# jfjell/Octree-Raymarcher

Measured on AMD Instinct MI355X. Metric: Mrays/s (primary+shadow) at 1920x1080, depth-12 SVO, higher is better.
Workload: dtype f32; 1 GPU; c3_1080p_depth12_4x1x4_shadow; depth_per_chunk=12, chunksize=128, nodes=99473656, bricks=34206642, hbm_pool_bytes=11087035656, kernel=auto, launches_in_flight=2, frames_per_launch=16, frames_in_flight=32, gather=False, partition=single, ranks_seen=1, launcher=single process

## Files before the change

### octree-raymarcher_amd/csrc/kernel_stack.hip.h

```cpp
#pragma once
#include "march.hip.h"
#include "step_asm.hip.h"

namespace svo {

constexpr int CW_ESCAPE_PENDING = (int)0x80000000;
enum : int { M_DONE = 0, M_WORLD = 1, M_HIT = 2, M_TREE = 3, M_TWIG = 4 };

constexpr int VOTE_WORLD = 8;
constexpr int VOTE_HIT = 16;
constexpr int VOTE_BUSY = 24;
constexpr int CREEP_SERIOUS = 6;
constexpr int CREEP_LANES = 8;
#define SVO_LIKELY(x) __builtin_expect(!!(x), 1)
#define SVO_UNLIKELY(x) __builtin_expect(!!(x), 0)
constexpr int STEP_EXTRA = 4;
constexpr int STEP_LANES = 8;
constexpr int DRAIN_STEPS = 8;
#ifndef SVO_SURE_MISS_WHEN
#define SVO_SURE_MISS_WHEN __builtin_amdgcn_readfirstlane(more ? 0 : 1)
#endif

__device__ __forceinline__ float recip_pow2(float x) { return __uint_as_float(0x7F000000u - __float_as_uint(x)); }

__device__ __forceinline__ int chunk_index_pow2(const TraceArgs &A, V3 p)
{
    float qx = p.x * A.inv_chunksize, qy = p.y * A.inv_chunksize, qz = p.z * A.inv_chunksize;
    if (qx < 0.0f) qx -= 1.0f;
    if (qy < 0.0f) qy -= 1.0f;
    if (qz < 0.0f) qz -= 1.0f;
    const int ix = (int)qx, iy = (int)qy, iz = (int)qz;
    const int rx = ix - A.ccm[0], ry = iy - A.ccm[1], rz = iz - A.ccm[2];
    int mx = A.cbase[0] + rx, my = A.cbase[1] + ry, mz = A.cbase[2] + rz;
    mx -= (mx >= A.dimw) ? A.dimw : 0; mx += (mx < 0) ? A.dimw : 0;
    my -= (my >= A.dimh) ? A.dimh : 0; my += (my < 0) ? A.dimh : 0;
    mz -= (mz >= A.dimd) ? A.dimd : 0; mz += (mz < 0) ? A.dimd : 0;
    return my * A.dimw * A.dimd + mz * A.dimw + mx;
}

__device__ __forceinline__ V3 cube_normal_pow2(V3 s, V3 lo, float size, float eps)
{
    const V3 hi = lo + size;
    const V3 c = (lo + hi) * 0.5f;
    const V3 p = s - c;
    const float d = fabsf(lo.x - hi.x) * 0.5f;
    const float invd = recip_pow2(d);
    const float b = 1.0f + eps;
    const float ix = (float)(int)((p.x * invd) * b), iy = (float)(int)((p.y * invd) * b), iz = (float)(int)((p.z * invd) * b);
    const float dot = ix * ix + iy * iy + iz * iz;
    float inv;
    if (dot == 1.0f) inv = 1.0f;
    else if (dot == 2.0f) inv = __uint_as_float(0x3F3504F3u);
    else if (dot == 3.0f) inv = __uint_as_float(0x3F13CD3Au);
    else inv = 1.0f / sqrtf(dot);
    return mk(ix * inv, iy * inv, iz * inv);
}

__device__ __forceinline__ uint32_t child_slot(int ux, int uy, int uz, int sh)
{
    const uint32_t bx = __builtin_amdgcn_ubfe((uint32_t)ux, (uint32_t)sh, 1u);
    const uint32_t by = __builtin_amdgcn_ubfe((uint32_t)uy, (uint32_t)sh, 1u);
    const uint32_t bz = __builtin_amdgcn_ubfe((uint32_t)uz, (uint32_t)sh, 1u);
    return ((bz << 1) + by) * 2u + bx;
}
__device__ __forceinline__ uint32_t ld_node(const uint32_t *pool, uint32_t boff)
{
    return *reinterpret_cast<const uint32_t *>(reinterpret_cast<const char *>(pool) + (size_t)boff);
}
constexpr uint32_t WIDE_PAYLOAD = (1u << 25) - 1u;
__device__ __forceinline__ uint32_t wide_slot(int ux, int uy, int uz, int sh)
{
    const uint32_t bx = __builtin_amdgcn_ubfe((uint32_t)ux, (uint32_t)sh, 2u);
    const uint32_t by = __builtin_amdgcn_ubfe((uint32_t)uy, (uint32_t)sh, 2u);
    const uint32_t bz = __builtin_amdgcn_ubfe((uint32_t)uz, (uint32_t)sh, 2u);
    return (bz << 4) | (by << 2) | bx;
}
__device__ __forceinline__ bool is_branch(uint32_t word) { return (int32_t)word < (int32_t)0xC0000000; }

__device__ __forceinline__ TraceArgs args_reloaded()
{
    auto p = __builtin_amdgcn_kernarg_segment_ptr();
    asm volatile("" : "+s"(p));
    TraceArgs T;
    __builtin_memcpy(&T, p, sizeof T);
    return T;
}
__device__ __forceinline__ FrameCam camera_reloaded(int f)
{
    auto p = __builtin_amdgcn_kernarg_segment_ptr();
    asm volatile("" : "+s"(p));
    FrameCam c;
    __builtin_memcpy(&c, (decltype(p))((const char __attribute__((address_space(4))) *)p + __builtin_offsetof(TraceArgs, cams) + (size_t)f * sizeof(FrameCam)), sizeof c);
    return c;
}

__device__ __noinline__ float brick_layer_first_touch(int k, V3 a, V3 b, V3 g, V3 bmin, float r, unsigned long long mask)
{
    const float ak = k == 0 ? a.x : k == 1 ? a.y : a.z, bk = k == 0 ? b.x : k == 1 ? b.y : b.z, mk_ = k == 0 ? bmin.x : k == 1 ? bmin.y : bmin.z;
    const float au = k == 0 ? a.y : k == 1 ? a.z : a.x, av = k == 0 ? a.z : k == 1 ? a.x : a.y;
    const float gu = k == 0 ? g.y : k == 1 ? g.z : g.x, gv = k == 0 ? g.z : k == 1 ? g.x : g.y;
    const float mu = k == 0 ? bmin.y : k == 1 ? bmin.z : bmin.x, mv = k == 0 ? bmin.z : k == 1 ? bmin.x : bmin.y;
    const int su = k == 0 ? 4 : k == 1 ? 16 : 1, sv = k == 0 ? 16 : k == 1 ? 1 : 4;
    const float delta = r * 0.0625f;
    bool ok = (ak == mk_) & (bk < 0.0f);
    ok &= (mu >= 4.0f * r) & (mv >= 4.0f * r) & (delta >= (fabsf(mu) + fabsf(mv) + 8.0f * r) * 0x1p-21f);
    ok = ok && fabsf(gu) < 1.0e30f && fabsf(gv) < 1.0e30f;
    if (!ok) return -1.0f;
    const float u0 = au - mu, v0 = av - mv;
    float first = __uint_as_float(0x7F800000u);
    bool clean = true;
    for (int cv = 0; cv < 4; ++cv) {
        const float va = ((float)cv * r - delta - v0) * gv, vb = ((float)(cv + 1) * r + delta - v0) * gv;
        const float v_in = fminf(va, vb), v_out = fmaxf(va, vb);
        for (int cu = 0; cu < 4; ++cu) {
            const bool occupied = (mask >> (cu * su + cv * sv)) & 1ull;
            const float ua = ((float)cu * r - delta - u0) * gu, ub = ((float)(cu + 1) * r + delta - u0) * gu;
            const float s_in = fmaxf(fmaxf(fminf(ua, ub), v_in), 0.0f), s_out = fminf(fmaxf(ua, ub), v_out);
            clean &= (s_in == s_in) & (s_out == s_out);
            first = (occupied & (s_in <= s_out)) ? fminf(first, s_in) : first;
        }
    }
    return clean ? first * (1.0f - 0x1p-18f) : -1.0f;
}

__device__ __forceinline__ void note_tile_cost(int outk, uint32_t steps)
{
    const TraceArgs T = args_reloaded();
    if (!T.tile_cost) return;
    const int k = outk & 0x7FFFFFFF;
    int tile, frame = 0;
    if (T.from_camera) {
        const int per = T.w * T.h;
        frame = k / per;
        const int r = k - frame * per;
        const int ly = r / T.w, lx = r - ly * T.w;
        tile = (ly / TILE_H) * T.tiles_per_row + lx / TILE_W;
    } else tile = k >> 6;
    atomicMax(&T.tile_cost[((size_t)frame * (size_t)T.ntiles + (size_t)tile) * 2 + (outk < 0 ? 1 : 0)], steps);
}

template <bool GLSL>
__device__ __forceinline__ bool past_far_end(int mode, float t, float tt_saved, float tw, float eps, float far)
{
    const float tt = mode == M_TWIG ? tt_saved : t;
    return (mode == M_TREE || mode == M_TWIG) && tw + (GLSL ? tt : tt - eps) >= far;
}

template <int MAXLV, int REFILL, int WAVES_PER_SIMD, bool BIG, bool GLSL, bool SEG = false>
__global__ __launch_bounds__(64, WAVES_PER_SIMD) void k_trace_stack(TraceArgs A)
{
    __shared__ uint32_t stk[MAXLV / 2 + 1][64];
    __shared__ float tile_ray[SEG ? 12 : 11][64];
    constexpr int CHUNK_TAB = (BIG && MAXLV <= 10) ? 128 : 64;
    __shared__ uint32_t chunk_tab[6][CHUNK_TAB];
    stk[0][threadIdx.x] = 0u;
    const int lane = threadIdx.x;
    const bool want_cost = A.tile_cost != nullptr;
    const int n_chunks = A.dimw * A.dimh * A.dimd;
    const bool chunks_in_lds = n_chunks <= CHUNK_TAB;
    if (chunks_in_lds)
        for (int i = lane; i < n_chunks; i += 64) {
            const DevWide ch = A.wchunks[i];
            chunk_tab[0][i] = __float_as_uint(ch.bmin[0]); chunk_tab[1][i] = __float_as_uint(ch.bmin[1]); chunk_tab[2][i] = __float_as_uint(ch.bmin[2]);
            chunk_tab[3][i] = ch.levels; chunk_tab[4][i] = ch.wide_off; chunk_tab[5][i] = (uint32_t)ch.twig_off;
        }
    __syncthreads();
#ifdef SVO_STACK_TIMING
    const unsigned long long t_begin = __builtin_amdgcn_s_memrealtime();
    unsigned n_iters = 0, n_tree_lanes = 0, n_twig_lanes = 0, n_world_lanes = 0;
    unsigned n_world_runs = 0, n_hit_runs = 0, n_refill = 0, n_tilegen = 0, n_fix = 0;
    unsigned n_lane_twig = 0;
    unsigned n_lane_busy = 0;
    unsigned n_creep_runs = 0, n_creep_rounds = 0, n_dbg = 0;
    unsigned n_wsteps = 0, n_lsteps = 0, n_hit_wait = 0, n_dead_wait = 0, n_wsteps_b = 0, n_lsteps_b = 0, n_world_wait = 0, n_twig_b = 0;
#endif
    [[maybe_unused]] StepStats step_stats;

    const V3 wlo = ld3(A.worldmin), whi = ld3(A.worldmax);
    const V3 sdir = ld3(A.sdir);
    const V3 sg = recip(sdir);
    const float eps = A.eps;
    const bool eps_pow2 = (__float_as_uint(eps) & 0x807FFFFFu) == 0u && __float_as_uint(eps) >= 0x00800000u && __float_as_uint(eps) < 0x7F800000u;
    const float csize = A.chunksize;

    const int tr_cols = A.tiles_per_row;
    const int tr_rows = A.ntiles / (tr_cols > 0 ? tr_cols : 1);
    const bool by_cols = tr_cols >= TILE_REGIONS;
    const int reg_q = (by_cols ? tr_cols : tr_rows) / TILE_REGIONS, reg_rem = (by_cols ? tr_cols : tr_rows) % TILE_REGIONS;
    int region = (int)(__builtin_amdgcn_s_getreg(20 | (0 << 6) | (3 << 11)) & (TILE_REGIONS - 1));
    int regions_left = TILE_REGIONS;
    int tile_first = 0;
    int tile_next = 64;
    bool more = true;
    unsigned rays_marched = 0;

    int mode = M_DONE;
    int outk = 0;
    V3 alpha = mk(0, 0, 0), beta = mk(0, 0, 1), g = mk(0, 0, 0);
    float tw = 0.0f;
    [[maybe_unused]] float far = __uint_as_float(0x7F800000u);
    int cw = 0;
    uint32_t guard = 0;
    V3 O = mk(0, 0, 0), Blo = mk(0, 0, 0);
    float res = 1.0f, t = 0.0f;
    int cnt = 0;
    float tt_saved = 0.0f, t_miss = 0.0f;
    int it_saved = 0;
    V3 clo = mk(0, 0, 0);
    WideRef<BIG> wide_b = 0;
    auto ld_wide = [&](uint32_t e) -> uint32_t {
        if constexpr (BIG) return *reinterpret_cast<const uint32_t *>((size_t)wide_b + ((size_t)e << 2));
        else return ld_node(A.wide, wide_b + (e << 2));
    };
    uint32_t twig_off = 0;
    int levels = 0, ci = -1;
    int pux = 0, puy = 0, puz = 0, valid = 0, plev = 0;
    unsigned long long bmask = 0;
#ifndef SVO_CXX_STEP
    float bsize = 0.0f, res_tree = 1.0f;
    int nw_chunk = 1;
    const uint32_t lds_lane = (uint32_t)(size_t)(__attribute__((address_space(3))) uint32_t *)&stk[0][lane];
    StepUniform SU;
    SU.csize = csize; SU.eps = eps; SU.eps2 = 2.0f * eps; SU.cap_twig = A.cap_twig; SU.wide = A.wide; SU.mask = A.mask; SU.descend_shift = MAXLV <= 10 ? DESCEND_SHIFT_SHALLOW : DESCEND_SHIFT_DEEP;
#endif
    int creepn = 0;
    for (;;) {
        unsigned long long dead = __ballot(mode == M_DONE);
        while (more && __popcll(dead) >= REFILL) {
            if (tile_next >= 64) {
                int t32 = -1, tcol = 0, trow = 0, tframe = 0;
                const uint32_t *order = args_reloaded().tile_order;
                if (order) {
                    regions_left = 0;
                    unsigned long long tix = 0;
                    if (lane == 0) tix = atomicAdd(&A.work[WORK_CURSOR0], 1ull);
                    int t = __builtin_amdgcn_readfirstlane((int)tix);
                    if (t < A.ntiles * A.nframes) {
                        tframe = t / A.ntiles; t -= tframe * A.ntiles;
                        t32 = (int)order[t];
                        if ((uint32_t)t32 >= (uint32_t)A.ntiles) { t32 = 0; tframe = -1; }
                        trow = t32 / tr_cols; tcol = t32 - trow * tr_cols;
                    }
                }
                while (regions_left > 0) {
                    const int span = reg_q + (region < reg_rem ? 1 : 0);
                    const int first = region * reg_q + (region < reg_rem ? region : reg_rem);
                    const int count = span * (by_cols ? tr_rows : tr_cols);
                    unsigned long long tix = 0;
                    if (lane == 0) tix = atomicAdd(&A.work[WORK_CURSOR0 + region], 1ull);
                    int t = __builtin_amdgcn_readfirstlane((int)tix);
                    if (t < count * A.nframes) {
                        if (A.nframes > 1) { tframe = t / count; t -= tframe * count; }
                        if (by_cols) { trow = t / span; tcol = first + (t - trow * span); }
                        else { trow = first + t / tr_cols; tcol = t % tr_cols; }
                        t32 = trow * tr_cols + tcol;
                        break;
                    }
                    region = (region + 1) & (TILE_REGIONS - 1);
                    --regions_left;
                }
                if (t32 < 0) { more = false; break; }
                tile_first = t32 * 64;
                tile_next = 0;
#ifdef SVO_STACK_TIMING
                ++n_tilegen;
#endif
                {
                    const TraceArgs T = args_reloaded();
                    const int id = tile_first + lane;
                    bool ok;
                    int k = -1;
                    V3 o = mk(0, 0, 0), d = mk(0, 0, 1);
                    if (T.from_camera) {
                        const int lx = tcol * TILE_W + (lane & (TILE_W - 1));
                        const int ly = trow * TILE_H + lane / TILE_W;
                        ok = (lx < T.w) & (ly < T.h) & (tframe >= 0);
                        k = (tframe * T.h + ly) * T.w + lx;
                        int px = 0, py = 0;
                        if (ok) local_to_pixel(T, lx, ly, px, py);
                        if (ok && (py >= T.imgh || px >= T.imgw)) { store_miss(A.out, k, 0); ok = false; }
                        if (ok) camera_ray(camera_reloaded(tframe), T.imgw, T.imgh, px, py, o, d);
                    } else {
                        ok = id < T.n && tframe >= 0;
                        k = id;
                        if (ok) { o = ld3(T.origins + 3 * (long long)id); d = ld3(T.dirs + 3 * (long long)id); }
                        if constexpr (SEG) tile_ray[11][lane] = ok ? T.tmax[id] : 0.0f;
                    }
                    const V3 gg = recip(d);
                    float t0 = 0.0f;
                    if (ok) {
                        bool hit = true;
                        if (!inside(o, wlo, whi)) t0 = (GLSL ? enter_glsl(o, gg, wlo, whi, hit) : enter(o, d, wlo, whi, hit)) + eps;
                        rays_marched++;
                        if (!hit) { store_miss(A.out, k, 0); ok = false; }
                    }
                    tile_ray[0][lane] = o.x; tile_ray[1][lane] = o.y; tile_ray[2][lane] = o.z;
                    tile_ray[3][lane] = d.x; tile_ray[4][lane] = d.y; tile_ray[5][lane] = d.z;
                    tile_ray[6][lane] = gg.x; tile_ray[7][lane] = gg.y; tile_ray[8][lane] = gg.z;
                    tile_ray[9][lane] = t0;
                    tile_ray[10][lane] = __int_as_float(ok ? k : -1);
                    __syncthreads();
                }
            }
#ifdef SVO_STACK_TIMING
            ++n_refill;
#endif
            const int rank = (int)__builtin_amdgcn_mbcnt_hi((unsigned)(dead >> 32), __builtin_amdgcn_mbcnt_lo((unsigned)dead, 0u));
            const int avail = 64 - tile_next;
            if (mode == M_DONE && rank < avail) {
                const int slot = tile_next + rank;
                const int k = __float_as_int(tile_ray[10][slot]);
                if (k >= 0) {
                    outk = k;
                    alpha = mk(tile_ray[0][slot], tile_ray[1][slot], tile_ray[2][slot]);
                    beta = mk(tile_ray[3][slot], tile_ray[4][slot], tile_ray[5][slot]);
                    g = mk(tile_ray[6][slot], tile_ray[7][slot], tile_ray[8][slot]);
                    tw = tile_ray[9][slot];
                    if constexpr (SEG) far = tile_ray[11][slot];
                    cw = 0; guard = 0; creepn = 0;
                    mode = M_WORLD;
                }
            }
            const int ndead = __popcll(dead);
            tile_next += (ndead < avail) ? ndead : avail;
            __syncthreads();
            dead = __ballot(mode == M_DONE);
        }
        if (dead == ~0ull) break;
#ifdef SVO_STACK_TIMING
        ++n_iters;
        n_tree_lanes += __popcll(__ballot(mode == M_TREE)); n_twig_lanes += __popcll(__ballot(mode == M_TWIG));
        n_world_lanes += __popcll(__ballot(mode == M_WORLD));
#endif

        const int n_busy = __popcll(__ballot(mode == M_TREE || mode == M_TWIG));
        const int n_world = __popcll(__ballot(mode == M_WORLD));
        const int n_hit = __popcll(__ballot(mode == M_HIT));
        const bool run_world = n_world > 0 && (n_world >= VOTE_WORLD || n_busy < VOTE_BUSY ||
                                               __ballot(mode == M_WORLD && creepn <= -CREEP_SERIOUS) != 0ull);
        const bool run_hit = n_hit > 0 && (n_hit >= VOTE_HIT || n_busy < VOTE_BUSY);

        if (SVO_UNLIKELY(mode != M_DONE && mode != M_HIT && ++guard > STEP_GUARD)) {
            if (outk < 0) store_flags(A.out, outk & 0x7FFFFFFF, SVO_HIT_FLAG | SVO_SHADOW_TRACED | SVO_ERR_FLAG | (A.normal_mode == SVO_NORMAL_FACE ? (uint32_t)SVO_FACE_NORMAL : 0u));
            else store_miss(A.out, outk, SVO_ERR_FLAG);
            mode = M_DONE;
        }

#ifdef SVO_STACK_TIMING
        n_world_runs += run_world; n_hit_runs += run_hit;
#endif
        if (run_world && mode == M_WORLD) {
            if (cw < 0) {
                cw &= ~CW_ESCAPE_PENDING;
                if constexpr (GLSL) tw += guarded(escape(O, g, clo, clo + csize), eps) + eps;
                else tw += escape(O, g, clo, clo + csize) + eps;
            }
            bool miss = cw >= A.cap_chunk;
            if constexpr (SEG) miss |= (GLSL ? tw : tw - eps) >= far;
            if (!miss) {
                cw++;
                const V3 p = alpha + beta * tw;
                miss = !inside(p, wlo, whi);
                if (!miss) {
                    const int ci_new = chunk_index_pow2(A, p);
                    if (ci_new != ci) { valid = 0; pux = 0; puy = 0; puz = 0; }
                    ci = ci_new;
                    uint32_t ch_levels, ch_wide, ch_twig;
                    if (chunks_in_lds) {
                        clo = mk(__uint_as_float(chunk_tab[0][ci]), __uint_as_float(chunk_tab[1][ci]), __uint_as_float(chunk_tab[2][ci]));
                        ch_levels = chunk_tab[3][ci]; ch_wide = chunk_tab[4][ci]; ch_twig = chunk_tab[5][ci];
                    } else {
                        const DevWide ch = A.wchunks[ci];
                        clo = ld3(ch.bmin);
                        ch_levels = ch.levels; ch_wide = ch.wide_off; ch_twig = (uint32_t)ch.twig_off;
                    }
                    bool contained = inside(p, clo, clo + csize);
                    if (GLSL && !contained) tw += guarded(escape(p, g, clo, clo + csize), eps) + eps;
                    else miss = !contained;
                    if (contained) {
                        if constexpr (BIG) wide_b = (unsigned long long)(size_t)A.wide + ((unsigned long long)ch_wide << 8);
                        else wide_b = ch_wide << 8;
                        twig_off = ch_twig;
                        levels = (int)ch_levels;
                        O = p; t = 0.0f; cnt = A.cap_tree;
                        Blo = clo;
                        res = csize * __uint_as_float((uint32_t)(127 - levels) << 23);
#ifndef SVO_CXX_STEP
                        bsize = csize; res_tree = res; nw_chunk = levels ? (levels + 1) >> 1 : 1;
#endif
                        mode = M_TREE;
                    }
                }
            }
            if (miss) {
                if (outk >= 0) store_miss(A.out, outk, 0);
                if (want_cost) note_tile_cost(outk, guard);
                mode = M_DONE;
            }
        }

        int pass = 0;
        const int fixed_steps = (n_busy >= STEP_LANES && __ballot(creepn > 0 || creepn <= -4 * CREEP_SERIOUS) == 0ull) ? STEP_EXTRA : 0;
        for (;;) {
#ifdef SVO_STACK_TIMING
        n_lane_twig += mode == M_TWIG ? (pass == 0 ? 1u + (unsigned)fixed_steps : (unsigned)DRAIN_STEPS) : 0u;
        n_lane_busy += (mode == M_TREE || mode == M_TWIG) ? (pass == 0 ? 1u + (unsigned)fixed_steps : (unsigned)DRAIN_STEPS) : 0u;
        { const int nm = __popcll(__ballot(mode == M_TREE || mode == M_TWIG)); n_wsteps += nm > 0; n_lsteps += nm; if (more) { n_wsteps_b += nm > 0; n_lsteps_b += nm; n_hit_wait += __popcll(__ballot(mode == M_HIT)); n_dead_wait += __popcll(__ballot(mode == M_DONE)); n_world_wait += __popcll(__ballot(mode == M_WORLD)); n_twig_b += __popcll(__ballot(mode == M_TWIG)); } }
#endif
#ifndef SVO_CXX_STEP
        const int nsteps = pass == 0 ? 1 + fixed_steps : DRAIN_STEPS;
        const int sure_miss = SVO_SURE_MISS_WHEN;
        march_steps_asm<BIG, GLSL>(mode, O, Blo, bsize, res, t, cnt, tt_saved, t_miss, it_saved, tw, cw, pux, puy, puz, valid, plev, bmask, creepn,
                                   beta, g, clo, alpha, levels, nw_chunk, res_tree, wide_b, twig_off, lds_lane, SU, nsteps | (sure_miss << 16), step_stats);
        pass += nsteps - 1;
#else
        if (mode == M_TREE || mode == M_TWIG) {
            enum : int { S_LEAVE = 0, S_ADVANCE = 1, S_ENTER = 2, S_HIT_LEAF = 3, S_HIT_CELL = 4, S_BAD = 5 };
            const bool twig = mode == M_TWIG;
            const float Bsize = twig ? res * 4.0f : csize, inv_res = recip_pow2(res);
            const int crept = creepn < 0 ? -creepn : creepn;
            creepn = -crept;
            bool leave = cnt <= 0;
            cnt -= 1;
            const V3 p = O + beta * t;
            leave |= !inside(p, Blo, Blo + Bsize);
            const float fx = (p.x - Blo.x) * inv_res, fy = (p.y - Blo.y) * inv_res, fz = (p.z - Blo.z) * inv_res;
            int ux = (int)fx, uy = (int)fy, uz = (int)fz;
#ifdef SVO_STACK_TIMING
            n_fix += __ballot(!twig && ((fx == (float)ux) | (fy == (float)uy) | (fz == (float)uz))) != 0;
#endif
            if (SVO_UNLIKELY(!twig && ((fx == (float)ux) | (fy == (float)uy) | (fz == (float)uz)))) {
                const int nmax = (1 << levels) - 1;
                ux = ux > nmax ? nmax : ux; uy = uy > nmax ? nmax : uy; uz = uz > nmax ? nmax : uz;
                ux -= (Blo.x + (float)ux * res > p.x) ? 1 : 0;
                uy -= (Blo.y + (float)uy * res > p.y) ? 1 : 0;
                uz -= (Blo.z + (float)uz * res > p.z) ? 1 : 0;
            }
            if (twig) leave |= (ux > 3) | (uy > 3) | (uz > 3);

            int what = S_LEAVE;
            int low = 0;
            uint32_t payload = 0;
            if (SVO_LIKELY(!leave)) {
                if (!twig) {
                    const uint32_t diff = (uint32_t)((ux ^ pux) | (uy ^ puy) | (uz ^ puz));
                    const int nw = levels ? (levels + 1) >> 1 : 1;
                    const int hb = 32 - __clz((int)(diff | 1u));
                    const int keep = nw - ((hb + 1) >> 1);
                    int k;
                    asm("v_med3_i32 %0, %1, 0, %2" : "=v"(k) : "v"(keep), "v"(valid));
                    uint32_t wnode = stk[k][lane];
                    int sh = 2 * (nw - 1 - k);
                    uint32_t word = ld_wide((wnode << 6) + wide_slot(ux, uy, uz, sh));
                    while (is_branch(word)) {
                        wnode = word & WIDE_PAYLOAD;
                        ++k;
                        stk[k][lane] = wnode;
                        sh -= 2;
                        word = ld_wide((wnode << 6) + wide_slot(ux, uy, uz, sh));
                    }
                    valid = k; pux = ux; puy = uy; puz = uz;
                    plev = (int)((word >> 25) & 31u);
                    low = (1 << (levels - plev)) - 1;
                    const uint32_t type = node_type(word);
                    what = type == EMPTY ? S_ADVANCE : type == LEAF ? S_HIT_LEAF : S_ENTER;
                    payload = word;
                } else {
                    payload = (uint32_t)(uz * 16 + uy * 4 + ux);
                    what = ((bmask >> payload) & 1ull) ? S_HIT_CELL : S_ADVANCE;
                }
            }

            if (what == S_ADVANCE || what == S_ENTER) {
                const V3 E_lo = mk(Blo.x + (float)(ux & ~low) * res, Blo.y + (float)(uy & ~low) * res, Blo.z + (float)(uz & ~low) * res);
                const float E_size = res * (float)(low + 1);
                const float e = (GLSL ? guarded(escape(p, g, E_lo, E_lo + E_size), eps) : escape(p, g, E_lo, E_lo + E_size)) + eps;
                if (what == S_ADVANCE) {
                    t += e;
                    creepn = e < 2.0f * eps ? crept + 1 : 0;
                } else {
                    bmask = A.mask[twig_off + (payload & WIDE_PAYLOAD)];
                    tt_saved = t; t_miss = t + e; it_saved = cnt;
                    O = p; t = 0.0f; cnt = A.cap_twig;
                    Blo = E_lo;
                    res = E_size * 0.25f;
                    mode = M_TWIG;
                }
            }
            if (leave) {
                if (twig) {
                    t = t_miss;
                    cnt = it_saved;
                    O = alpha + beta * tw;
                    Blo = clo;
                    res = csize * __uint_as_float((uint32_t)(127 - levels) << 23);
                    mode = M_TREE;
                } else {
                    cw |= CW_ESCAPE_PENDING;
                    mode = M_WORLD;
                }
            }
            if (what == S_HIT_LEAF) {
                tw = tw + (GLSL ? t : t - eps);
                cnt = (int)SVO_CELL_NONE;
                mode = M_HIT;
            }
            if (what == S_HIT_CELL) {
                float sdist = t;
                sdist += tt_saved;
                tw = tw + sdist;
                cnt = (int)payload;
                mode = M_HIT;
            }
        }
#endif

        ++pass;
        if (pass <= fixed_steps) continue;
        if (more || pass >= 256) break;
        const unsigned long long marching = __ballot(mode == M_TREE || mode == M_TWIG);
        if (marching == 0ull || marching != __ballot(mode != M_DONE) || __ballot(creepn > 0 || creepn <= -4 * CREEP_SERIOUS) != 0ull) break;
        if constexpr (SEG) if (__ballot(past_far_end<GLSL>(mode, t, tt_saved, tw, eps, far)) != 0ull) break;
        }
        guard += pass - 1;
        if constexpr (SEG) {
            if (past_far_end<GLSL>(mode, t, tt_saved, tw, eps, far)) {
                if (mode == M_TWIG) O = alpha + beta * tw;
                creepn = creepn > 0 ? -creepn : creepn;
                cw |= CW_ESCAPE_PENDING;
                mode = M_WORLD;
            }
        }

#include "creep_block.inc"

        if (mode == M_HIT && outk < 0) {
            store_flags(A.out, outk & 0x7FFFFFFF, SVO_HIT_FLAG | SVO_SHADOW_TRACED | SVO_SHADOWED | (A.normal_mode == SVO_NORMAL_FACE ? (uint32_t)SVO_FACE_NORMAL : 0u));
            if (want_cost) note_tile_cost(outk, guard);
            mode = M_DONE;
        }
        if constexpr (SEG) {
            if (mode == M_HIT && !(tw < far)) {
                store_miss(A.out, outk, 0);
                if (want_cost) note_tile_cost(outk, guard);
                mode = M_DONE;
            }
        }
        if (run_hit && mode == M_HIT) {
            const int nw = levels ? (levels + 1) >> 1 : 1;
            const uint32_t wn = valid > 0 ? stk[valid][lane] : 0u, slot = wide_slot(pux, puy, puz, 2 * (nw - 1 - valid));
            const uint32_t word = ld_wide((wn << 6) + slot);
            uint32_t node = 0u;
            if (plev != 0) {
                const uint32_t ci = ((slot >> 1) & 1u) | ((slot >> 2) & 2u) | ((slot >> 3) & 4u);
                const uint32_t gi = (slot & 1u) | ((slot >> 1) & 2u) | ((slot >> 2) & 4u);
                size_t wnode_in_pool;
                if constexpr (BIG) wnode_in_pool = (((size_t)wide_b - (size_t)A.wide) >> 8) + wn;
                else wnode_in_pool = (wide_b >> 8) + wn;
                const uint32_t *wb = A.wbase + wnode_in_pool * WIDE_BASE_WORDS;
                const int level_child = 2 * valid + 1 - (2 * nw - levels);
                node = plev == level_child ? wb[0] + ci : wb[1 + ci] + gi;
            }
            const uint32_t hitc = (uint32_t)cnt;
            V3 vlo;
            float vsize;
            uint32_t material;
            if (hitc == SVO_CELL_NONE) {
                const int low = (1 << (levels - plev)) - 1;
                vlo = mk(Blo.x + (float)(pux & ~low) * res, Blo.y + (float)(puy & ~low) * res, Blo.z + (float)(puz & ~low) * res);
                vsize = res * (float)(low + 1);
                material = word & 0xFFFFu;
            } else {
                vlo = mk(Blo.x + (float)(hitc & 3u) * res, Blo.y + (float)((hitc >> 2) & 3u) * res, Blo.z + (float)(hitc >> 4) * res);
                vsize = res;
                const unsigned long long brick = (unsigned long long)twig_off + (word & WIDE_PAYLOAD);
                material = A.bmat[brick];
                if (material == 0xFFFFu) material = A.twig[brick * TWIG_WORDS + hitc];
            }
            const V3 point = alpha + beta * (tw - eps);
            const bool face = A.normal_mode == SVO_NORMAL_FACE;
            const V3 n = face ? face_normal(point, vlo, vlo + vsize, beta) : cube_normal_pow2(point, vlo, vsize, eps);
            const uint32_t flags = SVO_HIT_FLAG | (A.shadow ? SVO_SHADOW_TRACED : 0u) | (face ? (uint32_t)SVO_FACE_NORMAL : 0u);
            store_hit(A.out, outk, tw, n, material, flags, (uint32_t)ci, node, hitc);
            if (want_cost) note_tile_cost(outk, guard);
            mode = M_DONE;
            if (A.shadow) {
                alpha = point; beta = sdir; g = sg;
                outk |= (int)0x80000000;
                if constexpr (SEG) far = __uint_as_float(0x7F800000u);
                tw = 0.0f; cw = 0; guard = 0; creepn = 0;
                bool hit = true;
                if (!inside(alpha, wlo, whi)) tw = (GLSL ? enter_glsl(alpha, g, wlo, whi, hit) : enter(alpha, beta, wlo, whi, hit)) + eps;
                mode = hit ? M_WORLD : M_DONE;
                rays_marched++;
            }
        }
    }

    unsigned total = rays_marched;
    for (int off = 32; off > 0; off >>= 1) total += __shfl_down(total, off, 64);
    if (lane == 0 && total) atomicAdd(&A.work[1], (unsigned long long)total);
#ifdef SVO_STACK_TIMING
    unsigned busiest = n_lane_busy;
    for (int off = 32; off > 0; off >>= 1) busiest = max(busiest, (unsigned)__shfl_xor((int)busiest, off, 64));
    unsigned busiest_twig = n_lane_busy == busiest ? n_lane_twig : 0u;
    for (int off = 32; off > 0; off >>= 1) busiest_twig = max(busiest_twig, (unsigned)__shfl_xor((int)busiest_twig, off, 64));
    if (lane == 0 && A.counters) {
        uint4 c; c.x = (uint32_t)t_begin; c.y = (uint32_t)__builtin_amdgcn_s_memrealtime(); c.z = n_iters; c.w = total;
        reinterpret_cast<uint4 *>(A.counters)[6 * blockIdx.x] = c;
        uint4 e; e.x = n_world_runs | (n_hit_runs << 16); e.y = n_refill | (n_tilegen << 12) | (n_fix << 20); e.z = n_tree_lanes; e.w = n_twig_lanes | (n_world_lanes << 20);
        reinterpret_cast<uint4 *>(A.counters)[6 * blockIdx.x + 1] = e;
        uint4 f; f.x = n_creep_runs | (busiest_twig << 16); f.y = busiest; f.z = n_creep_rounds; f.w = n_dbg;
        reinterpret_cast<uint4 *>(A.counters)[6 * blockIdx.x + 2] = f;
        uint4 h; h.x = n_wsteps; h.y = n_lsteps; h.z = n_hit_wait; h.w = n_dead_wait;
        reinterpret_cast<uint4 *>(A.counters)[6 * blockIdx.x + 3] = h;
        uint4 h2; h2.x = n_wsteps_b; h2.y = n_lsteps_b; h2.z = n_world_wait; h2.w = n_twig_b;
        reinterpret_cast<uint4 *>(A.counters)[6 * blockIdx.x + 4] = h2;
        uint4 h3; h3.x = step_stats.steps; h3.y = step_stats.lanes; h3.z = step_stats.stalls; h3.w = step_stats.chased;
        reinterpret_cast<uint4 *>(A.counters)[6 * blockIdx.x + 5] = h3;
    }
#endif
}

}
```

### octree-raymarcher_amd/csrc/march.hip.h

```cpp
#pragma once
#include <hip/hip_runtime.h>
#include "svo_format.h"
#include "../../include/svo.h"

namespace svo {

struct V3 { float x, y, z; };

__device__ __forceinline__ V3 mk(float x, float y, float z) { V3 r; r.x = x; r.y = y; r.z = z; return r; }
__device__ __forceinline__ V3 ld3(const float *p) { return mk(p[0], p[1], p[2]); }
__device__ __forceinline__ V3 operator+(V3 a, V3 b) { return mk(a.x + b.x, a.y + b.y, a.z + b.z); }
__device__ __forceinline__ V3 operator-(V3 a, V3 b) { return mk(a.x - b.x, a.y - b.y, a.z - b.z); }
__device__ __forceinline__ V3 operator*(V3 a, V3 b) { return mk(a.x * b.x, a.y * b.y, a.z * b.z); }
__device__ __forceinline__ V3 operator/(V3 a, V3 b) { return mk(a.x / b.x, a.y / b.y, a.z / b.z); }
__device__ __forceinline__ V3 operator+(V3 a, float s) { return mk(a.x + s, a.y + s, a.z + s); }
__device__ __forceinline__ V3 operator*(V3 a, float s) { return mk(a.x * s, a.y * s, a.z * s); }
__device__ __forceinline__ V3 operator/(V3 a, float s) { return mk(a.x / s, a.y / s, a.z / s); }

__device__ __forceinline__ float gmin(float x, float y) { return (y < x) ? y : x; }
__device__ __forceinline__ float gmax(float x, float y) { return (x < y) ? y : x; }

__device__ __forceinline__ bool inside(V3 p, V3 lo, V3 hi)
{
    return (p.x >= lo.x) & (p.y >= lo.y) & (p.z >= lo.z) & (hi.x >= p.x) & (hi.y >= p.y) & (hi.z >= p.z);
}

__device__ __forceinline__ float escape(V3 a, V3 g, V3 lo, V3 hi)
{
    const V3 t0 = (lo - a) * g, t1 = (hi - a) * g;
    const float tx = gmax(t0.x, t1.x), ty = gmax(t0.y, t1.y), tz = gmax(t0.z, t1.z);
    return gmin(tx, gmin(ty, tz));
}

constexpr float GLSL_BIGEPS = 0.0625f;
__device__ __forceinline__ float guarded(float d, float thr) { return d < thr ? GLSL_BIGEPS : d; }

__device__ __forceinline__ float enter_glsl(V3 a, V3 g, V3 lo, V3 hi, bool &hit)
{
    const V3 t0 = (lo - a) * g, t1 = (hi - a) * g;
    const float n0 = gmin(t0.x, t1.x), n1 = gmin(t0.y, t1.y), n2 = gmin(t0.z, t1.z);
    const float f0 = gmax(t0.x, t1.x), f1 = gmax(t0.y, t1.y), f2 = gmax(t0.z, t1.z);
    const float tnear = gmax(gmax(n0, n1), n2);
    const float tfar = gmin(gmin(f0, f1), f2);
    hit = (tfar > tnear) & (tnear > 0.0f);
    return tnear;
}

__device__ __forceinline__ float enter(V3 a, V3 b, V3 lo, V3 hi, bool &hit)
{
    const V3 t0 = (lo - a) / b, t1 = (hi - a) / b;
    const float n0 = gmin(t0.x, t1.x), n1 = gmin(t0.y, t1.y), n2 = gmin(t0.z, t1.z);
    const float f0 = gmax(t0.x, t1.x), f1 = gmax(t0.y, t1.y), f2 = gmax(t0.z, t1.z);
    const float tnear = gmax(gmax(n0, n1), n2);
    const float tfar = gmin(gmin(f0, f1), f2);
    hit = tfar > tnear;
    return tnear;
}

__device__ __forceinline__ V3 recip(V3 b) { return mk(1.0f / b.x, 1.0f / b.y, 1.0f / b.z); }
__device__ __forceinline__ V3 normalize3(V3 v)
{
    const float d = v.x * v.x + v.y * v.y + v.z * v.z;
    return v * (1.0f / sqrtf(d));
}

__device__ __forceinline__ V3 cube_normal(V3 s, V3 lo, V3 hi, float eps)
{
    const V3 c = (lo + hi) * 0.5f;
    const V3 p = s - c;
    const V3 dd = lo - hi;
    const V3 d = mk(fabsf(dd.x), fabsf(dd.y), fabsf(dd.z)) * 0.5f;
    const V3 n = (p / d) * (1.0f + eps);
    return normalize3(mk((float)(int)n.x, (float)(int)n.y, (float)(int)n.z));
}

__device__ __forceinline__ V3 face_normal(V3 s, V3 lo, V3 hi, V3 beta)
{
    const V3 c = (lo + hi) * 0.5f;
    const V3 p = s - c;
    const float ax = fabsf(p.x), ay = fabsf(p.y), az = fabsf(p.z);
    int k = 0; float pk = p.x, bk = beta.x, ak = ax;
    if (ay > ak) { k = 1; pk = p.y; bk = beta.y; ak = ay; }
    if (az > ak) { k = 2; pk = p.z; bk = beta.z; ak = az; }
    const float sgn = pk > 0.0f ? 1.0f : pk < 0.0f ? -1.0f : (bk > 0.0f ? -1.0f : 1.0f);
    return mk(k == 0 ? sgn : 0.0f, k == 1 ? sgn : 0.0f, k == 2 ? sgn : 0.0f);
}

__device__ __forceinline__ int pmod(int n, int m) { return (m + (n % m)) % m; }

__device__ __forceinline__ int chunk_index(const TraceArgs &A, V3 p)
{
    float qx = p.x / A.chunksize, qy = p.y / A.chunksize, qz = p.z / A.chunksize;
    if (qx < 0.0f) qx -= 1.0f;
    if (qy < 0.0f) qy -= 1.0f;
    if (qz < 0.0f) qz -= 1.0f;
    const int ix = (int)qx, iy = (int)qy, iz = (int)qz;
    return pmod(iy, A.dimh) * A.dimw * A.dimd + pmod(iz, A.dimd) * A.dimw + pmod(ix, A.dimw);
}

__device__ __forceinline__ void camera_ray(const FrameCam &c, int imgw, int imgh, int px, int py, V3 &o, V3 &d)
{
    const float fx = (float)px + 0.5f, fy = (float)py + 0.5f;
    const float u = ((fx / (float)imgw) * 2.0f - 1.0f) * c.tanx;
    const float v = (1.0f - (fy / (float)imgh) * 2.0f) * c.tany;
    const V3 dir = (ld3(c.fwd) + ld3(c.right) * u) + ld3(c.up) * v;
    d = normalize3(dir);
    o = ld3(c.eye);
}

__device__ __forceinline__ void local_to_pixel(const TraceArgs &A, int lx, int ly, int &px, int &py)
{
    px = A.x0 + lx;
    py = A.y0 + (ly / A.bh) * A.ystep + (ly % A.bh);
}

__device__ __forceinline__ void leaf_uv(V3 p, V3 cmin, float bsize, uint32_t m, float eps, float &u, float &v)
{
    const V3 cmax = cmin + bsize;
    const float size = cmax.x - cmin.x;
    float a = 0.0f, b = 0.0f;
    if (fabsf(p.x - cmin.x) <= eps) { a = p.y - cmin.y; b = p.z - cmin.z; }
    if (fabsf(p.x - cmax.x) <= eps) { a = p.y - cmax.y; b = p.z - cmax.z; }
    if (fabsf(p.y - cmin.y) <= eps) { a = p.x - cmin.x; b = p.z - cmin.z; }
    if (fabsf(p.y - cmax.y) <= eps) { a = p.x - cmax.x; b = p.z - cmax.z; }
    if (fabsf(p.z - cmin.z) <= eps) { a = p.x - cmin.x; b = p.y - cmin.y; }
    if (fabsf(p.z - cmax.z) <= eps) { a = p.x - cmax.x; b = p.y - cmax.y; }
    a = fabsf(a) / size; b = fabsf(b) / size;
    a = a + (((a < 0.125f ? 1.0f : 0.0f) - (a > 0.125f ? 1.0f : 0.0f)) * eps) * 2.0f;
    b = b + (((b < 0.125f ? 1.0f : 0.0f) - (b > 0.125f ? 1.0f : 0.0f)) * eps) * 2.0f;
    u = ((float)(m & 0xFFu) + a) / 256.0f;
    v = ((float)((m >> 8) & 0xFFu) + b) / 256.0f;
}

struct Voxel { V3 lo; float size; uint32_t material, node, cell; };

__device__ __forceinline__ void store_hit(void *out, int64_t k, float t, V3 n, uint32_t material, uint32_t flags,
                                          uint32_t chunk, uint32_t node, uint32_t cell)
{
    uint4 a, b;
    a.x = __float_as_uint(t); a.y = __float_as_uint(n.x); a.z = __float_as_uint(n.y); a.w = __float_as_uint(n.z);
    b.x = (material & 0xFFFFu) | (flags << 16); b.y = chunk; b.z = node; b.w = cell;
    uint4 *rec = reinterpret_cast<uint4 *>(out) + 2 * k;
    rec[0] = a;
    rec[1] = b;
}
__device__ __forceinline__ void store_miss(void *out, int64_t k, uint32_t flags)
{
    uint4 z; z.x = z.y = z.z = z.w = 0u;
    uint4 b = z; b.x = flags << 16;
    uint4 *rec = reinterpret_cast<uint4 *>(out) + 2 * k;
    rec[0] = z;
    rec[1] = b;
}
__device__ __forceinline__ void store_flags(void *out, int64_t k, uint32_t flags)
{
    reinterpret_cast<uint16_t *>(out)[16 * k + 9] = (uint16_t)flags;
}

constexpr uint32_t STEP_GUARD = 1u << 22;

}
```

Before: 7355 Mrays/s.

## Defer hit shading into batched wave-wide resolve pass via LDS queue

Hit lanes now write raw traversal state (voxel coords, level, wide node, cell) straight into the output record and push their ray index onto an LDS queue, then immediately start their shadow ray. Once 64 hits have queued, the whole wave reloads those records, recomputes the camera ray and the voxel bounds, and writes the material, node and normal in one fully occupied pass. The aim is to stop running the divergent material and normal code with only a few active lanes. The cost is an extra global write and read per hit, recomputing the camera ray, and a smaller LDS chunk table that makes room for the queue.

```diff
diff --git a/octree-raymarcher_amd/csrc/hit_resolve.hip.h b/octree-raymarcher_amd/csrc/hit_resolve.hip.h
--- /dev/null
+++ b/octree-raymarcher_amd/csrc/hit_resolve.hip.h
@@ -0,0 +1,89 @@
+#pragma once
+
+namespace svo {
+
+__device__ __forceinline__ uint32_t ld_raw(const uint32_t *p) { return __hip_atomic_load(p, __ATOMIC_RELAXED, __HIP_MEMORY_SCOPE_AGENT); }
+
+__device__ __forceinline__ void resolve_hits(const uint32_t *queue, int n, const uint32_t *chunk_tab, int tab_stride)
+{
+    const TraceArgs T = args_reloaded();
+    const int lane = threadIdx.x;
+    const bool active = lane < n;
+    __builtin_amdgcn_fence(__ATOMIC_RELEASE, "workgroup");
+    __builtin_amdgcn_fence(__ATOMIC_ACQUIRE, "workgroup");
+    if (active) {
+        const int k = (int)queue[lane];
+        uint32_t *rec = reinterpret_cast<uint32_t *>(T.out) + 8 * (size_t)k;
+        const float tw = __uint_as_float(ld_raw(rec + 0));
+        const int pux = (int)ld_raw(rec + 1), puy = (int)ld_raw(rec + 2), puz = (int)ld_raw(rec + 3);
+        const uint32_t packed = ld_raw(rec + 4);
+        const uint32_t ci = ld_raw(rec + 5), wn = ld_raw(rec + 6), hitc = ld_raw(rec + 7);
+        const int plev = (int)(packed & 0xFFu), valid = (int)((packed >> 8) & 0xFFu);
+
+        V3 o = mk(0, 0, 0), d = mk(0, 0, 1);
+        if (T.from_camera) {
+            const int per = T.w * T.h;
+            const int frame = k / per;
+            const int r = k - frame * per;
+            const int ly = r / T.w, lx = r - ly * T.w;
+            int px = 0, py = 0;
+            local_to_pixel(T, lx, ly, px, py);
+            bool todo = true;
+            while (todo) {
+                const int f = __builtin_amdgcn_readfirstlane(frame);
+                if (frame == f) {
+                    camera_ray(camera_reloaded(f), T.imgw, T.imgh, px, py, o, d);
+                    todo = false;
+                }
+            }
+        } else {
+            o = ld3(T.origins + 3 * (long long)k);
+            d = ld3(T.dirs + 3 * (long long)k);
+        }
+
+        V3 clo;
+        uint32_t ch_levels, ch_wide, ch_twig;
+        if (chunk_tab) {
+            clo = mk(__uint_as_float(chunk_tab[ci]), __uint_as_float(chunk_tab[tab_stride + ci]), __uint_as_float(chunk_tab[2 * tab_stride + ci]));
+            ch_levels = chunk_tab[3 * tab_stride + ci]; ch_wide = chunk_tab[4 * tab_stride + ci]; ch_twig = chunk_tab[5 * tab_stride + ci];
+        } else {
+            const DevWide ch = T.wchunks[ci];
+            clo = ld3(ch.bmin);
+            ch_levels = ch.levels; ch_wide = ch.wide_off; ch_twig = (uint32_t)ch.twig_off;
+        }
+        const int levels = (int)ch_levels;
+        const float res_tree = T.chunksize * __uint_as_float((uint32_t)(127 - levels) << 23);
+        const int low = (1 << (levels - plev)) - 1;
+        V3 vlo = mk(clo.x + (float)(pux & ~low) * res_tree, clo.y + (float)(puy & ~low) * res_tree, clo.z + (float)(puz & ~low) * res_tree);
+        float vsize = res_tree * (float)(low + 1);
+
+        const int nw = levels ? (levels + 1) >> 1 : 1;
+        const uint32_t slot = wide_slot(pux, puy, puz, 2 * (nw - 1 - valid));
+        const size_t wnode_in_pool = (size_t)ch_wide + wn;
+        const uint32_t word = T.wide[(wnode_in_pool << 6) + slot];
+        uint32_t node = 0u;
+        if (plev != 0) {
+            const uint32_t cix = ((slot >> 1) & 1u) | ((slot >> 2) & 2u) | ((slot >> 3) & 4u);
+            const uint32_t gi = (slot & 1u) | ((slot >> 1) & 2u) | ((slot >> 2) & 4u);
+            const uint32_t *wb = T.wbase + wnode_in_pool * WIDE_BASE_WORDS;
+            const int level_child = 2 * valid + 1 - (2 * nw - levels);
+            node = plev == level_child ? wb[0] + cix : wb[1 + cix] + gi;
+        }
+        uint32_t material;
+        if (hitc == SVO_CELL_NONE) material = word & 0xFFFFu;
+        else {
+            vsize = vsize * 0.25f;
+            vlo = mk(vlo.x + (float)(hitc & 3u) * vsize, vlo.y + (float)((hitc >> 2) & 3u) * vsize, vlo.z + (float)(hitc >> 4) * vsize);
+            const unsigned long long brick = (unsigned long long)ch_twig + (word & WIDE_PAYLOAD);
+            material = T.bmat[brick];
+            if (material == 0xFFFFu) material = T.twig[brick * TWIG_WORDS + hitc];
+        }
+        const V3 point = o + d * (tw - T.eps);
+        const V3 nrm = T.normal_mode == SVO_NORMAL_FACE ? face_normal(point, vlo, vlo + vsize, d) : cube_normal_pow2(point, vlo, vsize, T.eps);
+        store_hit_normal(T.out, k, nrm);
+        store_hit_material_node(T.out, k, material, node);
+    }
+}
+
+
+}
diff --git a/octree-raymarcher_amd/csrc/kernel_stack.hip.h b/octree-raymarcher_amd/csrc/kernel_stack.hip.h
--- a/octree-raymarcher_amd/csrc/kernel_stack.hip.h
+++ b/octree-raymarcher_amd/csrc/kernel_stack.hip.h
@@ -8,7 +8,9 @@
 enum : int { M_DONE = 0, M_WORLD = 1, M_HIT = 2, M_TREE = 3, M_TWIG = 4 };
 
 constexpr int VOTE_WORLD = 8;
-constexpr int VOTE_HIT = 16;
+constexpr int VOTE_HIT = 1;
+constexpr int RESOLVE_AT = 64;
+constexpr int HIT_QUEUE = 128;
 constexpr int VOTE_BUSY = 24;
 constexpr int CREEP_SERIOUS = 6;
 constexpr int CREEP_LANES = 8;
@@ -139,6 +141,10 @@
     atomicMax(&T.tile_cost[((size_t)frame * (size_t)T.ntiles + (size_t)tile) * 2 + (outk < 0 ? 1 : 0)], steps);
 }
 
+}
+#include "hit_resolve.hip.h"
+namespace svo {
+
 template <bool GLSL>
 __device__ __forceinline__ bool past_far_end(int mode, float t, float tt_saved, float tw, float eps, float far)
 {
@@ -151,8 +157,9 @@
 {
     __shared__ uint32_t stk[MAXLV / 2 + 1][64];
     __shared__ float tile_ray[SEG ? 12 : 11][64];
-    constexpr int CHUNK_TAB = (BIG && MAXLV <= 10) ? 128 : 64;
+    constexpr int CHUNK_TAB = (BIG && MAXLV <= 10) ? 104 : MAXLV > 16 ? 40 : 64;
     __shared__ uint32_t chunk_tab[6][CHUNK_TAB];
+    __shared__ uint32_t hit_queue[HIT_QUEUE];
     stk[0][threadIdx.x] = 0u;
     const int lane = threadIdx.x;
     const bool want_cost = A.tile_cost != nullptr;
@@ -167,8 +174,9 @@
     __syncthreads();
 #ifdef SVO_STACK_TIMING
     const unsigned long long t_begin = __builtin_amdgcn_s_memrealtime();
-    unsigned n_iters = 0, n_tree_lanes = 0, n_twig_lanes = 0, n_world_lanes = 0;
+    unsigned n_iters = 0, n_twig_lanes = 0, n_world_lanes = 0;
     unsigned n_world_runs = 0, n_hit_runs = 0, n_refill = 0, n_tilegen = 0, n_fix = 0;
+    unsigned n_resolve_calls = 0, n_resolved = 0;
     unsigned n_lane_twig = 0;
     unsigned n_lane_busy = 0;
     unsigned n_creep_runs = 0, n_creep_rounds = 0, n_dbg = 0;
@@ -193,6 +201,7 @@
     int tile_next = 64;
     bool more = true;
     unsigned rays_marched = 0;
+    int n_queued = 0;
 
     int mode = M_DONE;
     int outk = 0;
@@ -329,16 +338,14 @@
         if (dead == ~0ull) break;
 #ifdef SVO_STACK_TIMING
         ++n_iters;
-        n_tree_lanes += __popcll(__ballot(mode == M_TREE)); n_twig_lanes += __popcll(__ballot(mode == M_TWIG));
+        n_twig_lanes += __popcll(__ballot(mode == M_TWIG));
         n_world_lanes += __popcll(__ballot(mode == M_WORLD));
 #endif
 
         const int n_busy = __popcll(__ballot(mode == M_TREE || mode == M_TWIG));
         const int n_world = __popcll(__ballot(mode == M_WORLD));
-        const int n_hit = __popcll(__ballot(mode == M_HIT));
         const bool run_world = n_world > 0 && (n_world >= VOTE_WORLD || n_busy < VOTE_BUSY ||
                                                __ballot(mode == M_WORLD && creepn <= -CREEP_SERIOUS) != 0ull);
-        const bool run_hit = n_hit > 0 && (n_hit >= VOTE_HIT || n_busy < VOTE_BUSY);
 
         if (SVO_UNLIKELY(mode != M_DONE && mode != M_HIT && ++guard > STEP_GUARD)) {
             if (outk < 0) store_flags(A.out, outk & 0x7FFFFFFF, SVO_HIT_FLAG | SVO_SHADOW_TRACED | SVO_ERR_FLAG | (A.normal_mode == SVO_NORMAL_FACE ? (uint32_t)SVO_FACE_NORMAL : 0u));
@@ -347,7 +354,7 @@
         }
 
 #ifdef SVO_STACK_TIMING
-        n_world_runs += run_world; n_hit_runs += run_hit;
+        n_world_runs += run_world;
 #endif
         if (run_world && mode == M_WORLD) {
             if (cw < 0) {
@@ -546,55 +553,50 @@
                 mode = M_DONE;
             }
         }
-        if (run_hit && mode == M_HIT) {
-            const int nw = levels ? (levels + 1) >> 1 : 1;
-            const uint32_t wn = valid > 0 ? stk[valid][lane] : 0u, slot = wide_slot(pux, puy, puz, 2 * (nw - 1 - valid));
-            const uint32_t word = ld_wide((wn << 6) + slot);
-            uint32_t node = 0u;
-            if (plev != 0) {
-                const uint32_t ci = ((slot >> 1) & 1u) | ((slot >> 2) & 2u) | ((slot >> 3) & 4u);
-                const uint32_t gi = (slot & 1u) | ((slot >> 1) & 2u) | ((slot >> 2) & 4u);
-                size_t wnode_in_pool;
-                if constexpr (BIG) wnode_in_pool = (((size_t)wide_b - (size_t)A.wide) >> 8) + wn;
-                else wnode_in_pool = (wide_b >> 8) + wn;
-                const uint32_t *wb = A.wbase + wnode_in_pool * WIDE_BASE_WORDS;
-                const int level_child = 2 * valid + 1 - (2 * nw - levels);
-                node = plev == level_child ? wb[0] + ci : wb[1 + ci] + gi;
-            }
-            const uint32_t hitc = (uint32_t)cnt;
-            V3 vlo;
-            float vsize;
-            uint32_t material;
-            if (hitc == SVO_CELL_NONE) {
-                const int low = (1 << (levels - plev)) - 1;
-                vlo = mk(Blo.x + (float)(pux & ~low) * res, Blo.y + (float)(puy & ~low) * res, Blo.z + (float)(puz & ~low) * res);
-                vsize = res * (float)(low + 1);
-                material = word & 0xFFFFu;
-            } else {
-                vlo = mk(Blo.x + (float)(hitc & 3u) * res, Blo.y + (float)((hitc >> 2) & 3u) * res, Blo.z + (float)(hitc >> 4) * res);
-                vsize = res;
-                const unsigned long long brick = (unsigned long long)twig_off + (word & WIDE_PAYLOAD);
-                material = A.bmat[brick];
-                if (material == 0xFFFFu) material = A.twig[brick * TWIG_WORDS + hitc];
-            }
-            const V3 point = alpha + beta * (tw - eps);
-            const bool face = A.normal_mode == SVO_NORMAL_FACE;
-            const V3 n = face ? face_normal(point, vlo, vlo + vsize, beta) : cube_normal_pow2(point, vlo, vsize, eps);
-            const uint32_t flags = SVO_HIT_FLAG | (A.shadow ? SVO_SHADOW_TRACED : 0u) | (face ? (uint32_t)SVO_FACE_NORMAL : 0u);
-            store_hit(A.out, outk, tw, n, material, flags, (uint32_t)ci, node, hitc);
-            if (want_cost) note_tile_cost(outk, guard);
-            mode = M_DONE;
-            if (A.shadow) {
-                alpha = point; beta = sdir; g = sg;
-                outk |= (int)0x80000000;
-                if constexpr (SEG) far = __uint_as_float(0x7F800000u);
-                tw = 0.0f; cw = 0; guard = 0; creepn = 0;
-                bool hit = true;
-                if (!inside(alpha, wlo, whi)) tw = (GLSL ? enter_glsl(alpha, g, wlo, whi, hit) : enter(alpha, beta, wlo, whi, hit)) + eps;
-                mode = hit ? M_WORLD : M_DONE;
-                rays_marched++;
-            }
-        }
+        const unsigned long long hits = __ballot(mode == M_HIT);
+        if (hits != 0ull && (VOTE_HIT <= 1 || __popcll(hits) >= VOTE_HIT || n_busy < VOTE_BUSY)) {
+#ifdef SVO_STACK_TIMING
+            ++n_hit_runs;
+#endif
+            if (mode == M_HIT) {
+                const uint32_t wn = valid > 0 ? stk[valid][lane] : 0u;
+                const bool face = A.normal_mode == SVO_NORMAL_FACE;
+                const uint32_t flags = SVO_HIT_FLAG | (A.shadow ? SVO_SHADOW_TRACED : 0u) | (face ? (uint32_t)SVO_FACE_NORMAL : 0u);
+                store_hit(A.out, outk, tw, mk(__int_as_float(pux), __int_as_float(puy), __int_as_float(puz)), (uint32_t)(plev | (valid << 8)), flags,
+                          (uint32_t)ci, wn, (uint32_t)cnt);
+                const int rank = (int)__builtin_amdgcn_mbcnt_hi((unsigned)(hits >> 32), __builtin_amdgcn_mbcnt_lo((unsigned)hits, 0u));
+                hit_queue[n_queued + rank] = (uint32_t)outk;
+                if (want_cost) note_tile_cost(outk, guard);
+                mode = M_DONE;
+                if (A.shadow) {
+                    alpha = alpha + beta * (tw - eps); beta = sdir; g = sg;
+                    outk |= (int)0x80000000;
+                    if constexpr (SEG) far = __uint_as_float(0x7F800000u);
+                    tw = 0.0f; cw = 0; guard = 0; creepn = 0;
+                    bool hit = true;
+                    if (!inside(alpha, wlo, whi)) tw = (GLSL ? enter_glsl(alpha, g, wlo, whi, hit) : enter(alpha, beta, wlo, whi, hit)) + eps;
+                    mode = hit ? M_WORLD : M_DONE;
+                    rays_marched++;
+                }
+            }
+            n_queued += __popcll(hits);
+            if (SVO_UNLIKELY(n_queued >= RESOLVE_AT)) {
+                const int take = n_queued < 64 ? n_queued : 64;
+#ifdef SVO_STACK_TIMING
+                ++n_resolve_calls; n_resolved += (unsigned)take;
+#endif
+                resolve_hits(hit_queue, take, chunks_in_lds ? &chunk_tab[0][0] : nullptr, CHUNK_TAB);
+                const uint32_t rest = hit_queue[(64 + lane) & (HIT_QUEUE - 1)];
+                n_queued -= take;
+                if (lane < n_queued) hit_queue[lane] = rest;
+            }
+        }
+    }
+    if (n_queued > 0) {
+#ifdef SVO_STACK_TIMING
+        ++n_resolve_calls; n_resolved += (unsigned)n_queued;
+#endif
+        resolve_hits(hit_queue, n_queued, chunks_in_lds ? &chunk_tab[0][0] : nullptr, CHUNK_TAB);
     }
 
     unsigned total = rays_marched;
@@ -608,7 +610,7 @@
     if (lane == 0 && A.counters) {
         uint4 c; c.x = (uint32_t)t_begin; c.y = (uint32_t)__builtin_amdgcn_s_memrealtime(); c.z = n_iters; c.w = total;
         reinterpret_cast<uint4 *>(A.counters)[6 * blockIdx.x] = c;
-        uint4 e; e.x = n_world_runs | (n_hit_runs << 16); e.y = n_refill | (n_tilegen << 12) | (n_fix << 20); e.z = n_tree_lanes; e.w = n_twig_lanes | (n_world_lanes << 20);
+        uint4 e; e.x = n_world_runs | (n_hit_runs << 16); e.y = n_refill | (n_tilegen << 12) | (n_fix << 20); e.z = n_resolved | (n_resolve_calls << 20); e.w = n_twig_lanes | (n_world_lanes << 20);
         reinterpret_cast<uint4 *>(A.counters)[6 * blockIdx.x + 1] = e;
         uint4 f; f.x = n_creep_runs | (busiest_twig << 16); f.y = busiest; f.z = n_creep_rounds; f.w = n_dbg;
         reinterpret_cast<uint4 *>(A.counters)[6 * blockIdx.x + 2] = f;
diff --git a/octree-raymarcher_amd/csrc/march.hip.h b/octree-raymarcher_amd/csrc/march.hip.h
--- a/octree-raymarcher_amd/csrc/march.hip.h
+++ b/octree-raymarcher_amd/csrc/march.hip.h
@@ -156,6 +156,16 @@
 {
     reinterpret_cast<uint16_t *>(out)[16 * k + 9] = (uint16_t)flags;
 }
+__device__ __forceinline__ void store_hit_normal(void *out, int64_t k, V3 n)
+{
+    float *rec = reinterpret_cast<float *>(out) + 8 * k;
+    rec[1] = n.x; rec[2] = n.y; rec[3] = n.z;
+}
+__device__ __forceinline__ void store_hit_material_node(void *out, int64_t k, uint32_t material, uint32_t node)
+{
+    reinterpret_cast<uint16_t *>(out)[16 * k + 8] = (uint16_t)material;
+    reinterpret_cast<uint32_t *>(out)[8 * k + 6] = node;
+}
 
 constexpr uint32_t STEP_GUARD = 1u << 22;
 
```

Result: slower. 5929 Mrays/s (-19.4%).
